# bigai-nlco/VideoTGB

Measured on AMD Instinct MI355X. Metric: clips/sec end-to-end VideoQA (96->8 frames), higher is better.
Workload: dtype bf16; 1 GPU; InstructBLIP-Vicuna-7B + TGB, T=96->8 of 32 frames, 224x224, greedy 16 new tokens (BASELINE.json configs[2]); inputs=resident in HBM when the timed region starts, global_batch=124, parallelism=clip-parallel x1 (no data-path collective), streams=1, weights=seeded N(0,0.02) random init

## Files before the change

include/vtgb.h:

```cpp
#ifndef VTGB_H
#define VTGB_H

#include <stddef.h>
#include <stdint.h>

#ifdef __cplusplus
extern "C" {
#endif

typedef struct ihipStream_t* vtgb_stream_t;

#define VTGB_VERSION 601

#define VTGB_OK 0
#define VTGB_EINVAL (-1)
#define VTGB_EWORKSPACE (-2)
#define VTGB_EHIP (-3)
#define VTGB_EUNSUPPORTED (-4)

#define VTGB_F32 0
#define VTGB_BF16 1
#define VTGB_BF16X3 2
#define VTGB_F16C8 3

// ... 360 lines not shown
    int32_t n_images, H, W;
    int32_t variant;
    int32_t out_kind;
    const void* x;
    const void* weights;
    const float* bias;
    const int32_t* scale;
    const void* resid;
    void* out;
    float* moments;
    void* workspace;
    size_t workspace_bytes;
} vtgb_raft_layer1_h8_args;
size_t vtgb_raft_layer1_h8_workspace_bytes(const vtgb_raft_layer1_h8_args* a);
int vtgb_raft_layer1_h8(const vtgb_raft_layer1_h8_args* a, vtgb_stream_t stream);

typedef struct {
    int32_t dtype, n_pairs, H8, W8, dim;
    int32_t pairs_per_clip, frames_per_clip, first_off, second_off, n_images;
    float scale;
    const float* fmap;
    void* levels[4];
    void* workspace;
    size_t workspace_bytes;
} vtgb_raft_corr_args;
size_t vtgb_raft_corr_workspace_bytes(const vtgb_raft_corr_args* a);
int vtgb_raft_corr(const vtgb_raft_corr_args* a, vtgb_stream_t stream);

#define VTGB_RAFT_ENC_NW 40
typedef struct {
// ... 295 lines not shown
```

videotgb_amd/_lib.py:

```python
from __future__ import annotations

import ctypes as C
import os

import torch

HERE = os.path.dirname(os.path.abspath(__file__))
LIB_PATH = os.environ.get("VTGB_LIB") or os.path.join(HERE, "libvtgb.so")

F32, BF16 = 0, 1
BF16X3 = 2
F16C8 = 3
MAP_A, MAP_B = 0, 1
POOL_MEAN, POOL_CONCAT = 0, 1
TGB_MODE = {"text": 0, "vision": 0, "fusion": 1, "multi_modal": 2}
EPI_STORE, EPI_GELU, EPI_RESID_F32, EPI_STORE_F32 = 0, 1, 2, 3
VIT_NW_GLOBAL, VIT_NW_LAYER = 6, 18
QF_NW_GLOBAL, QF_NW_LAYER = 4, 32
TGB_NW_GLOBAL, TGB_NW_LAYER = 17, 26

EXPORTS = [
    "vtgb_version", "vtgb_last_error", "vtgb_pack_bf16", "vtgb_span_select", "vtgb_span_to_frames",
    "vtgb_gather_frames", "vtgb_vit_patch_kpad", "vtgb_vit_workspace_bytes", "vtgb_vit_forward",
    "vtgb_qformer_workspace_bytes", "vtgb_qformer_forward", "vtgb_pool_project_workspace_bytes",
# ... 7 lines not shown
    "vtgb_gemm_skinny_workspace_bytes", "vtgb_gemm_skinny", "vtgb_pack_skinny_weight_bytes", "vtgb_pack_skinny_weight",
    "vtgb_pack_skinny_weight_fp8_bytes", "vtgb_pack_skinny_weight_fp8", "vtgb_gemm_skinny_fp8", "vtgb_gemm_skinny_bias",
    "vtgb_raft_update_workspace_bytes", "vtgb_raft_update", "vtgb_raft_encoder_workspace_bytes", "vtgb_raft_encoder",
    "vtgb_raft_corr_workspace_bytes", "vtgb_raft_corr", "vtgb_preprocess_frames", "vtgb_concat_text_io", "vtgb_shifted_ce_forward", "vtgb_shifted_ce_backward",
    "vtgb_comm_unique_id", "vtgb_comm_init", "vtgb_comm_destroy", "vtgb_allreduce_f32",
    "vtgb_attn_train_forward", "vtgb_attn_train_backward",
    "vtgb_gemm_train", "vtgb_gemm_train_workspace_bytes", "vtgb_col_sum_parts", "vtgb_col_sum_f32", "vtgb_layernorm_train_partials", "vtgb_layernorm_train_forward", "vtgb_layernorm_train_backward",
    "vtgb_gelu_forward", "vtgb_gelu_backward",
    "vtgb_pair_pack", "vtgb_pair_conv", "vtgb_pair_conv_ex", "vtgb_attention_tiled",
    "vtgb_llm_decode_attention_split_workspace_bytes", "vtgb_llm_decode_attention_split",
    "vtgb_llm_decode_attention_split_fp8", "vtgb_llm_rope_cache_fp8", "vtgb_llm_rope_cache_prefill_fp8",
    "vtgb_raft_lookup_convc1", "vtgb_raft_gru_half", "vtgb_llm_lora", "vtgb_conv_launch", "vtgb_attention_cached",
    "vtgb_llm_decode_attention_beam", "vtgb_llm_beam_candidates", "vtgb_llm_attention_rows_beam", "vtgb_llm_decode_attention_beam_fp8",
    "vtgb_pack_skinny_weight_mxfp4_bytes", "vtgb_pack_skinny_weight_mxfp4", "vtgb_gemm_skinny_mxfp4",
    "vtgb_raft_stem_workspace_bytes", "vtgb_raft_stem", "vtgb_llm_lora_parts", "vtgb_llm_pick_greedy", "vtgb_llm_beam_candidates_eos",
    "vtgb_raft_layer1_h8_workspace_bytes", "vtgb_raft_layer1_h8",
]
COMM_ID_BYTES = 128

i32, i64, f32, vp, sz = C.c_int32, C.c_int64, C.c_float, C.c_void_p, C.c_size_t


class AttnTrainArgs(C.Structure):
    _fields_ = [("batch", i32), ("heads", i32), ("head_dim", i32), ("s_q", i32), ("s_kv", i32), ("q", vp), ("k", vp), ("v", vp),
                ("q_tok", i64), ("kv_tok", i64), ("q_batch", i64), ("kv_batch", i64), ("key_mask", vp), ("drop", vp), ("scale", f32),
                ("out", vp), ("o_tok", i64), ("o_batch", i64), ("lse", vp), ("dout", vp), ("dq", vp), ("dk", vp), ("dv", vp), ("delta", vp)]


class GemmTrainArgs(C.Structure):
    _fields_ = [("compute", i32), ("M", i32), ("N", i32), ("K", i32), ("a", vp), ("lda", i64), ("a_dtype", i32), ("a_kmajor", i32),
                ("b", vp), ("ldb", i64), ("b_dtype", i32), ("b_kmajor", i32), ("bias", vp), ("out", vp), ("ldo", i64), ("workspace", vp), ("workspace_bytes", sz)]
# ... 103 lines not shown
class ConvLaunchArgs(C.Structure):
    _fields_ = [("dtype", i32), ("out_kind", i32), ("site", i32), ("n_images", i32), ("H", i32), ("W", i32), ("KH", i32), ("KW", i32), ("stride", i32),
                ("Hi", i32), ("Wi", i32), ("C1", i32), ("C2", i32), ("N", i32), ("act", i32), ("post_relu", i32), ("out_scale", f32), ("a", vp), ("a2", vp),
                ("weights", vp), ("bias", vp), ("out", vp), ("ld_out", i64), ("moments", vp), ("stats_part", vp), ("stats_part_floats", i64), ("resid", vp),
                ("ld_resid", i64), ("tail_w", vp), ("tail_out", vp)]


class RaftStemArgs(C.Structure):
    _fields_ = [("n_images", i32), ("H", i32), ("W", i32), ("variant", i32), ("out_kind", i32), ("images", vp), ("weights", vp), ("bias", vp), ("out", vp),
                ("moments", vp), ("workspace", vp), ("workspace_bytes", sz)]


class RaftLayer1H8Args(C.Structure):
    _fields_ = [("n_images", i32), ("H", i32), ("W", i32), ("variant", i32), ("out_kind", i32), ("x", vp), ("weights", vp), ("bias", vp), ("scale", vp),
                ("resid", vp), ("out", vp), ("moments", vp), ("workspace", vp), ("workspace_bytes", sz)]


class RaftCorrArgs(C.Structure):
    _fields_ = [("dtype", i32), ("n_pairs", i32), ("H8", i32), ("W8", i32), ("dim", i32), ("pairs_per_clip", i32), ("frames_per_clip", i32),
                ("first_off", i32), ("second_off", i32), ("n_images", i32), ("scale", f32), ("fmap", vp), ("levels", vp * 4),
                ("workspace", vp), ("workspace_bytes", sz)]


class RaftEncoderArgs(C.Structure):
    _fields_ = [("dtype", i32), ("n_images", i32), ("H", i32), ("W", i32), ("norm", i32), ("images", vp), ("weights", C.POINTER(vp)), ("out", vp),
                ("workspace", vp), ("workspace_bytes", sz)]


class GemmSkinnyArgs(C.Structure):
    _fields_ = [("M", i32), ("N", i32), ("K", i32), ("n_splits", i32), ("x", vp), ("ldx", i64), ("w", vp), ("ldw", i64), ("out", vp), ("ldo", i64),
# ... 122 lines not shown
    L.vtgb_pair_conv_ex.restype = C.c_int
    L.vtgb_raft_lookup_convc1.argtypes = [C.POINTER(RaftLookupConvc1Args), vp]
    L.vtgb_raft_lookup_convc1.restype = C.c_int
    L.vtgb_raft_gru_half.argtypes = [C.POINTER(RaftGruHalfArgs), vp]
    L.vtgb_raft_gru_half.restype = C.c_int
    L.vtgb_conv_launch.argtypes = [C.POINTER(ConvLaunchArgs), vp]
    L.vtgb_conv_launch.restype = C.c_int
    L.vtgb_raft_stem.argtypes = [C.POINTER(RaftStemArgs), vp]
    L.vtgb_raft_stem.restype = C.c_int
    L.vtgb_raft_stem_workspace_bytes.argtypes = [C.POINTER(RaftStemArgs)]
    L.vtgb_raft_stem_workspace_bytes.restype = sz
    L.vtgb_raft_layer1_h8.argtypes = [C.POINTER(RaftLayer1H8Args), vp]
    L.vtgb_raft_layer1_h8.restype = C.c_int
    L.vtgb_raft_layer1_h8_workspace_bytes.argtypes = [C.POINTER(RaftLayer1H8Args)]
    L.vtgb_raft_layer1_h8_workspace_bytes.restype = sz
    L.vtgb_raft_update.argtypes = [C.POINTER(RaftUpdateArgs), vp]
    L.vtgb_raft_update.restype = C.c_int
    L.vtgb_raft_update_workspace_bytes.argtypes = [C.POINTER(RaftUpdateArgs)]
    L.vtgb_raft_update_workspace_bytes.restype = sz
    L.vtgb_raft_encoder.argtypes = [C.POINTER(RaftEncoderArgs), vp]
    L.vtgb_raft_encoder.restype = C.c_int
    L.vtgb_raft_encoder_workspace_bytes.argtypes = [C.POINTER(RaftEncoderArgs)]
    L.vtgb_raft_encoder_workspace_bytes.restype = sz
    L.vtgb_raft_corr.argtypes = [C.POINTER(RaftCorrArgs), vp]
    L.vtgb_raft_corr.restype = C.c_int
    L.vtgb_raft_corr_workspace_bytes.argtypes = [C.POINTER(RaftCorrArgs)]
    L.vtgb_raft_corr_workspace_bytes.restype = sz
    L.vtgb_llm_rmsnorm.argtypes = [C.c_int, vp, vp, vp, vp, i64, i32, f32, vp]
    L.vtgb_llm_rope_cache.argtypes = [C.c_int, vp, vp, vp, vp, vp, vp, vp, i32, i32, i32, i32, i32, vp]
    L.vtgb_llm_rope_cache_prefill.argtypes = [C.c_int, vp, vp, vp, vp, vp, i32, i32, i32, i32, i32, i32, vp]
# ... 123 lines not shown
```

videotgb_amd/csrc/common.h:

```cpp
#pragma once
#include <hip/hip_runtime.h>
#include <stdint.h>
#include <stdio.h>

#include "vtgb.h"

typedef __bf16 bf16_t;
typedef __attribute__((ext_vector_type(8))) __bf16 bf16x8;
typedef __attribute__((ext_vector_type(4))) __bf16 bf16x4;
typedef __attribute__((ext_vector_type(4))) float f32x4;

#if defined(__HIPCC__)
__device__ __forceinline__ float bf16_round(float v) {
    unsigned u = __float_as_uint(v);
    if ((u & 0x7F800000u) != 0x7F800000u) u += 0x7FFFu + ((u >> 16) & 1u);
    return __uint_as_float(u & 0xFFFF0000u);
}
#endif

void vtgb_set_error(const char* fmt, ...);

#define VTGB_REQUIRE(cond, code, ...)  \
    do {                               \
        if (!(cond)) {                 \
// ... 146 lines not shown
bool stem7x7_supported(int H, int W);
int launch_stem7x7(const float* img, const void* w, const float* bias, float* out_f32, float* stats, float* stats_part, void* out_bf16, int n_img, int H, int W,
                   int relu, hipStream_t s);
int launch_stem7x7_x3(const float* img, const void* w, const float* bias, float* out_f32, float* stats, float* stats_part, void* out_pair, int h8, int n_img, int H,
                      int W, hipStream_t s);
size_t conv64_stats_part_floats(int n_img);
int launch_stats_finish_tiles(const float* part, float* stats, int n_img, int HW, int N, int64_t M, hipStream_t s);
int launch_stats_finish_parts(const float* part, float* stats, int n_img, int parts, int C, hipStream_t s);
int cu_count();

bool conv3x3_c64_supported(int H, int W);
int launch_conv3x3_c64(const void* in, const void* w, const float* bias, float* out_f32, float* stats, float* stats_part, void* out_bf16, const void* resid,
                       int n_img, int H, int W, int relu, int post_relu, hipStream_t s);
bool layer1_h8_supported(int H, int W);
int launch_layer1_h8(const void* in, const void* w, const float* bias, const int* scale, float* out_f32, void* out_pair, const void* resid, int out_bf16, int n_img, int H,
                     int W, hipStream_t s);

struct LnDesc {
    int dtype, M, D;
    float eps;
    const float* x;
    int64_t ldx;
    RowMap x_map;
    const float* gamma;
    const float* beta;
    float* out_f32;
    void* out_act;
    int64_t ldo;
    RowMap o_map;
};
int launch_layernorm(const LnDesc& d, hipStream_t s);
// ... 27 lines not shown
```

videotgb_amd/csrc/conv64.hip:

```cpp
#include <type_traits>
#include <utility>
#include "common.h"
#include "pair_h8.h"

namespace {

constexpr int C64_R = 8, C64_RS = 128;
constexpr int C64_ROW_BYTES = C64_RS * 128;
constexpr int C64_LDS = C64_R * C64_ROW_BYTES + 8 * 32 * 2 * 4 + 64 * 4;
typedef __attribute__((address_space(3))) void* c64_lptr_t;

struct Conv64Params {
    const bf16_t* in;
    const bf16_t* w;
    const float* bias;
    float* out_f32;
    float* stats;
    float* stats_part;
    bf16_t* out_bf16;
    const bf16_t* resid;
    int n_img, H, W, relu, post_relu;
    int parts, rows_per_part;
};

// ... 414 lines not shown
typedef _Float16 l1_f16x8 __attribute__((ext_vector_type(8)));

template <class F, int... G>
__device__ __forceinline__ void l1_static_for(std::integer_sequence<int, G...>, F&& f) { (f(std::integral_constant<int, G>{}), ...); }

struct Layer1H8Params {
    const char* in;
    const char* w;
    const float* bias;
    const int* scale;
    float* out_f32;
    char* out_pair;
    const char* resid;
    int n_img, H, W, out_bf16;
    int parts, rows_per_part, row_bytes;
};

template <int MODE, int OBF>
__global__ __launch_bounds__(512) void layer1_h8_kernel(const Layer1H8Params p) {
#if defined(__HIP_DEVICE_COMPILE__)
    extern __shared__ __attribute__((aligned(16))) char ring[];
    const int tid = threadIdx.x, lane = tid & 63, fr = lane & 15, fg = lane >> 4;
    const int wave = __builtin_amdgcn_readfirstlane(tid >> 6);
    const int wn = wave & 3, wm = wave >> 2;
    const int H = p.H, W = p.W, row_bytes = p.row_bytes;
    const int sc_w = *p.scale;

    l1_i32x4 wh[9][2];
    l1_i32x8 wc[9];
    {
        const char* const wrow = p.w + (wn * 16 + fr) * 2304 + fg * 16;
#pragma unroll
        for (int t = 0; t < 9; t++) {
            wh[t][0] = *reinterpret_cast<const l1_i32x4*>(wrow + t * 128);
            wh[t][1] = *reinterpret_cast<const l1_i32x4*>(wrow + t * 128 + 64);
            wc[t].lo = *reinterpret_cast<const l1_i32x4*>(wrow + (9 + t) * 128);
            wc[t].hi = *reinterpret_cast<const l1_i32x4*>(wrow + (9 + t) * 128 + 64);
        }
    }
    float* const bias_s = reinterpret_cast<float*>(ring + (L1_R - 1) * row_bytes + L1_READ_SPAN);
    if (tid < 64) bias_s[tid] = p.bias[tid];
    __syncthreads();

    constexpr unsigned OOB = 0x80000000u;
    const int n_pieces = row_bytes >> 10;
    const int dma_x = wave * 4 + (lane >> 4) - 1;
    const unsigned dma_off0 = (unsigned)(dma_x * 256 + (((lane & 15) ^ ((dma_x + 1) & 15)) << 4));
    unsigned x_off[3];
#pragma unroll
    for (int kx = 0; kx < 3; kx++) {
        const int slot = wm * 64 + fr + kx;
        x_off[kx] = (unsigned)(slot * 256 + ((fg ^ (slot & 15)) << 4));
    }
    const int nj = W - wm * 64 >= 64 ? 4 : W - wm * 64 <= 0 ? 0 : (W - wm * 64 + 15) >> 4;
    typedef __attribute__((__vector_size__(4 * sizeof(unsigned)))) unsigned u32x4_t;
    typedef __attribute__((__vector_size__(2 * sizeof(unsigned)))) unsigned u32x2_t;
    constexpr int OPX = 256;
// ... 7 lines not shown
        if (y0 >= H) continue;
        const int y1 = y0 + p.rows_per_part < H ? y0 + p.rows_per_part : H;
        const int64_t ioff = (int64_t)img * H * W * 256;
        const auto rsrc = __builtin_amdgcn_make_buffer_rsrc(const_cast<char*>(p.in + ioff), 0, H * W * 256, 0x00020000);
        const auto orsrc = __builtin_amdgcn_make_buffer_rsrc(MODE == 0 ? (void*)(reinterpret_cast<char*>(p.out_f32) + ioff) : (void*)(p.out_pair + ioff), 0, H * W * OPX, 0x00020000);
        const auto rrsrc = __builtin_amdgcn_make_buffer_rsrc(const_cast<char*>((MODE == 2 ? p.resid : p.in) + ioff), 0, H * W * 256, 0x00020000);
#define L1_ISSUE(yy)                                                                                                          \
        {                                                                                                                      \
            const int so_ = ((yy) >= 0 && (yy) < H) ? (yy) * W * 256 : 0x7FFFFF00;        \
            char* const dst_ = ring + ((yy) & (L1_R - 1)) * row_bytes + wave * 1024;                                           \
            _Pragma("unroll") for (int q = 0; q < 4; q++)                                                                      \
                if (q * 8 + wave < n_pieces)                                                                                   \
                    __builtin_amdgcn_raw_ptr_buffer_load_lds(rsrc, (c64_lptr_t)(dst_ + q * 8192), 16,                          \
                                                             (dma_x + q * 32 >= 0 && dma_x + q * 32 < W) ? dma_off0 + q * 8192u : OOB, so_, 0, 0); \
        }
        __builtin_amdgcn_s_waitcnt(0x0F70);
        __builtin_amdgcn_s_barrier();
        L1_ISSUE(y0 - 1)
        L1_ISSUE(y0)
        L1_ISSUE(y0 + 1)
        auto step = [&](auto nj_c, const int y) {
            constexpr int NJ = decltype(nj_c)::value;
            constexpr int NST = (MODE == 0 ? 1 : 2) * NJ;
            if (y == y0) __builtin_amdgcn_s_waitcnt(0x0F70);
            else __builtin_amdgcn_s_waitcnt(0x0F70 | NST);
            __builtin_amdgcn_s_barrier();
            u32x2_t rh[NJ], rl[NJ];
            if constexpr (MODE == 2) {
#pragma unroll
                for (int jj = 0; jj < NJ; jj++) {
                    const unsigned off = px0 + jj * 16 < W ? o_off0 + (unsigned)(jj * 16 * OPX + y * W * 256) : OOB;
                    rh[jj] = __builtin_bit_cast(u32x2_t, __builtin_amdgcn_raw_buffer_load_b64(rrsrc, off, 0, 0));
                    rl[jj] = __builtin_bit_cast(u32x2_t, __builtin_amdgcn_raw_buffer_load_b64(rrsrc, off != OOB ? off + 128u : OOB, 0, 0));
                }
            }
            L1_ISSUE(y + 2)
            f32x4 acc[NJ];
#pragma unroll
            for (int jj = 0; jj < NJ; jj++) acc[jj] = *reinterpret_cast<const f32x4*>(bias_s + wn * 16 + fg * 4);
            l1_i32x4 xg[3][NJ];
// ... 48 lines not shown
                        hu = __builtin_bit_cast(u32x2_t, hi); lu = __builtin_bit_cast(u32x2_t, lo);
                    } else {
                        h8_split4(v, hu, lu);
                    }
                    __builtin_amdgcn_raw_buffer_store_b64(hu, orsrc, off, 0, 0);
                    __builtin_amdgcn_raw_buffer_store_b64(lu, orsrc, ok ? off + 128u : OOB, 0, 0);
                }
            }
        };
        if (nj == 3) {
            for (int y = y0; y < y1; y++) step(std::integral_constant<int, 3>{}, y);
        } else {
            for (int y = y0; y < y1; y++) step(std::integral_constant<int, 4>{}, y);
        }
#undef L1_ISSUE
    }
#endif
}

}

bool conv3x3_c64_supported(int H, int W) { return W >= 16 && W <= C64_RS - 2 && H >= 1; }

size_t conv64_stats_part_floats(int n_img) { return ((size_t)n_img + 4 * (size_t)cu_count()) * 2 * 64 * 2; }

int launch_conv3x3_c64(const void* in, const void* w, const float* bias, float* out_f32, float* stats, float* stats_part, void* out_bf16, const void* resid,
                       int n_img, int H, int W, int relu, int post_relu, hipStream_t s) {
    VTGB_REQUIRE(conv3x3_c64_supported(H, W), VTGB_EUNSUPPORTED, "conv3x3_c64: W=%d outside [16, %d]", W, C64_RS - 2);
    VTGB_REQUIRE((int64_t)H * W * 128 < 0x7FFFFF00ll, VTGB_EUNSUPPORTED, "conv3x3_c64: image too large");
    Conv64Params p;
// ... 67 lines not shown
}

int launch_stem7x7(const float* img, const void* w, const float* bias, float* out_f32, float* stats, float* stats_part, void* out_bf16, int n_img, int H, int W,
                   int relu, hipStream_t s) {
    return stem7x7_launch(false, img, w, bias, out_f32, stats, stats_part, out_bf16, 0, n_img, H, W, relu, s);
}
int launch_stem7x7_x3(const float* img, const void* w, const float* bias, float* out_f32, float* stats, float* stats_part, void* out_pair, int h8, int n_img, int H,
                      int W, hipStream_t s) {
    VTGB_REQUIRE((out_f32 != nullptr) != (out_pair != nullptr), VTGB_EINVAL, "stem7x7 x3: exactly one of the fp32 rows and the pair rows");
    return stem7x7_launch(true, img, w, bias, out_f32, stats, stats_part, out_pair, h8, n_img, H, W, out_pair ? 1 : 0, s);
}

bool layer1_h8_supported(int H, int W) { return W >= 16 && W <= L1_MAX_W && H >= 4 && (int64_t)H * W * 256 < 0x7FFFFF00ll; }

int launch_layer1_h8(const void* in, const void* w, const float* bias, const int* scale, float* out_f32, void* out_pair, const void* resid, int out_bf16, int n_img, int H,
                     int W, hipStream_t s) {
    VTGB_REQUIRE(n_img > 0 && layer1_h8_supported(H, W), VTGB_EUNSUPPORTED, "layer1_h8: %d images of %d x %d outside 16 <= W <= %d, H >= 4", n_img, H, W, L1_MAX_W);
    VTGB_REQUIRE(in && w && bias && scale && ((out_f32 != nullptr) != (out_pair != nullptr)) && (!resid || out_pair) && (!out_bf16 || resid), VTGB_EINVAL,
                 "layer1_h8: operands, the scale byte and exactly one of the fp32 rows and the pair rows (resid belongs to pair rows, bf16 pairs to the residual tail)");
    Layer1H8Params p;
    p.in = (const char*)in; p.w = (const char*)w; p.bias = bias; p.scale = scale; p.out_f32 = out_f32; p.out_pair = (char*)out_pair; p.resid = (const char*)resid;
    p.n_img = n_img; p.H = H; p.W = W; p.out_bf16 = out_bf16;
    p.row_bytes = ((W + 2 + 3) / 4) * 1024;
    int parts = 1;
    while ((int64_t)n_img * parts < 4 * cu_count() && H / (parts * 2) >= 7) parts *= 2;
    p.rows_per_part = (H + parts - 1) / parts;
    p.parts = (H + p.rows_per_part - 1) / p.rows_per_part;
    const int64_t units = (int64_t)n_img * p.parts;
    const int grid = units < cu_count() ? (int)units : cu_count();
    const int lds = (L1_R - 1) * p.row_bytes + L1_READ_SPAN + 256;
    constexpr int lds_max = (L1_R - 1) * ((L1_MAX_W + 2 + 3) / 4) * 1024 + L1_READ_SPAN + 256;
    const double flops = 2.0 * n_img * H * W * 64.0 * 576.0;
    ProfScope prof(VTGB_PROF_CONV, flops, s, 2.0 * flops);
    static DeviceOnce a0, a1, a2, a3;
    if (out_f32) {
        VTGB_FUNC_LDS_ONCE(a0, (layer1_h8_kernel<0, 0>), lds_max);
        hipLaunchKernelGGL((layer1_h8_kernel<0, 0>), dim3(grid), dim3(512), lds, s, p);
    } else if (!resid) {
        VTGB_FUNC_LDS_ONCE(a1, (layer1_h8_kernel<1, 0>), lds_max);
        hipLaunchKernelGGL((layer1_h8_kernel<1, 0>), dim3(grid), dim3(512), lds, s, p);
    } else if (!out_bf16) {
        VTGB_FUNC_LDS_ONCE(a2, (layer1_h8_kernel<2, 0>), lds_max);
        hipLaunchKernelGGL((layer1_h8_kernel<2, 0>), dim3(grid), dim3(512), lds, s, p);
    } else {
        VTGB_FUNC_LDS_ONCE(a3, (layer1_h8_kernel<2, 1>), lds_max);
        hipLaunchKernelGGL((layer1_h8_kernel<2, 1>), dim3(grid), dim3(512), lds, s, p);
    }
    VTGB_HIP(hipGetLastError());
    return VTGB_OK;
}
// ... 1 lines not shown
```

videotgb_amd/csrc/raft_enc.hip:

```cpp
#include <math.h>
#include <string.h>

#include "common.h"
#include "conv_descs.h"

template <typename T>
__global__ __launch_bounds__(256) void raft_stem_pack_kernel(const float* __restrict__ img, T* __restrict__ out, T* __restrict__ pad_page,
                                                             int64_t n_px, int H, int W) {
    constexpr bool PAIR = sizeof(T) == 2;
    constexpr int CP = PAIR ? 128 : 64;
    const int64_t i = (int64_t)blockIdx.x * blockDim.x + threadIdx.x;
    if (i < 64) pad_page[i] = (T)0.f;
    if (i >= n_px * 4) return;
    const int64_t px_i = i >> 2;
    const int dX = (int)(i & 3), W2 = W >> 1, H2 = H >> 1;
    const int X = (int)(px_i % W2), Y = (int)((px_i / W2) % H2);
    const int64_t n = px_i / ((int64_t)W2 * H2);
    T v[12], l[12];
#pragma unroll
    for (int py = 0; py < 2; py++)
#pragma unroll
        for (int pxx = 0; pxx < 2; pxx++) {
            const int col = 2 * (X + dX - 2) + pxx, row = 2 * Y + py;
            const bool ok = (unsigned)col < (unsigned)W;
// ... 223 lines not shown
    d.algo_flops = 2.0 * (double)M2 * 64 * 147;
    VTGB_TRY(launch_conv_gemm(d, s));
    if (t.pair) return launch_x3_pair_pass(t.cf, 64, nullptr, HW, nullptr, 128, 64, t.pair, 128, 64, 64, 64, 1, 0, M2, s, t.h8);
    if (sf) return launch_stats_finish_tiles(sf, t.stats, t.n, HW, 64, M2, s);
    const int splits = HW >= 4096 ? 16 : HW >= 1024 ? 4 : 1;
    hipLaunchKernelGGL(inorm_stats_kernel, dim3(t.n, splits), dim3(256), 0, s, t.cf, t.spart, HW, 64, 64);
    return launch_stats_finish_parts(t.spart, t.stats, t.n, splits, 64, s);
}

struct EncH8 {
    const void* A; const void* W; const float* bias; const int* scale;
    int n, H, Wd, C, Cpad;
    float* cf; float* spart; float* stats;
    void* pair; const void* resid; int out_bf16;
    void* zero;
};
static int g_l1_h8 = 3;
extern "C" void vtgb_debug_set_l1_h8(int mask) { g_l1_h8 = mask & 3; }
static int enc_conv_h8(const EncH8& t, int variant, hipStream_t s) {
    const int HW = t.H * t.Wd, C2 = 2 * t.Cpad;
    const int64_t Mo = (int64_t)t.n * HW;
    if (variant != 0) {
        VTGB_REQUIRE(t.C == 64 && t.Cpad == 64 && layer1_h8_supported(t.H, t.Wd), VTGB_EUNSUPPORTED, "enc_conv_h8: the row-resident kernel takes 64 -> 64 channels, 16 <= W <= 112, H >= 4");
        VTGB_REQUIRE(variant == 1 || (!t.pair && t.spart && HW >= 256), VTGB_EINVAL, "enc_conv_h8: tile-order moments belong to fp32 rows of images of >= 256 pixels");
        VTGB_TRY(launch_layer1_h8(t.A, t.W, t.bias, t.scale, t.pair ? nullptr : t.cf, t.pair, t.resid, t.out_bf16, t.n, t.H, t.Wd, s));
        if (variant == 1) return VTGB_OK;
        hipLaunchKernelGGL(stats_tiles_c64_kernel, dim3((unsigned)((Mo + 255) / 256)), dim3(512), 0, s, t.cf, t.spart, (int)Mo, HW);
        return launch_stats_finish_tiles(t.spart, t.stats, t.n, HW, 64, Mo, s);
    }
    GemmDesc d;
    memset(&d, 0, sizeof(d));
    d.dtype = VTGB_BF16; d.M = (int)Mo; d.K = 9 * C2;
    d.A = t.A; d.lda = C2; d.W = t.W; d.ldw = d.K; d.bias = t.bias;
    d.conv_H = t.H; d.conv_W = t.Wd; d.conv_KH = 3; d.conv_KW = 3; d.conv_Cin = C2; d.conv_split = C2; d.zero_page = t.zero;
    d.h8_run = 9 * (t.Cpad / 64); d.h8_scale = t.scale;
    d.algo_flops = 2.0 * Mo * (double)t.C * (9 * t.C);
    if (!t.pair) {
        d.N = t.C; d.epi = VTGB_EPI_STORE_F32; d.out = t.cf; d.ldo = t.Cpad;
        d.col_stats = t.spart; d.stats_rows = HW;
        VTGB_TRY(launch_conv_h8(d, s));
        if (t.spart) VTGB_TRY(launch_stats_finish_tiles(t.spart, t.stats, t.n, HW, t.C, Mo, s));
        return VTGB_OK;
    }
    d.N = t.Cpad; d.epi = VTGB_EPI_SPLIT; d.act = 1; d.out = t.pair; d.ldo = C2; d.split_lo = t.Cpad;
// ... 138 lines not shown
        } else if (!inorm && !x3) {
            VTGB_TRY(conv_bn(Mo, g, 3, Cin_pad, g.stride, Hi, Wi, x, bw[0], F(bw[1]), 1, nullptr, 0, t1));
            const void* res = x;
            outb = t2;
            if (g.stride != 1) {
                VTGB_TRY(conv_bn(Mo, g, 1, Cin_pad, g.stride, Hi, Wi, x, bw[4], F(bw[5]), 0, nullptr, 0, t2));
                res = t2;
                outb = x;
            }
            VTGB_TRY(conv_bn(Mo, g, 3, g.Cpad, 1, g.Ho, g.Wo, t1, bw[2], F(bw[3]), 1, res, 1, outb));
        } else if (h8l1) {
            VTGB_REQUIRE(w[40], VTGB_EINVAL, "raft_encoder: weights[40] (the f16c8 convolutions' scale bytes) is NULL at VTGB_F16C8");
            const int C2 = 2 * g.Cpad;
            const bool s2 = g.stride != 1;
            const bool l1 = g.C == 64 && g.Cpad == 64 && !s2 && layer1_h8_supported(g.Ho, g.Wo);
            auto conv_h8 = [&](const void* A, const void* Wt, const float* bias, float* col_stats, int si) -> int {
                const EncH8 t{A, Wt, bias, (const int*)w[40] + si, n, g.Ho, g.Wo, g.C, g.Cpad, cf, col_stats, stats, nullptr, nullptr, 0, zero};
                return enc_conv_h8(t, l1 && (g_l1_h8 & 2) ? (col_stats ? 2 : 1) : 0, s);
            };
            auto conv_pair = [&](const void* A, const void* Wt, const float* bias, int si, const void* resid, void* out, int out_bf16) -> int {
                const EncH8 t{A, Wt, bias, (const int*)w[40] + si, n, g.Ho, g.Wo, g.C, g.Cpad, nullptr, nullptr, nullptr, out, resid, out_bf16, zero};
                return enc_conv_h8(t, l1 && (g_l1_h8 & 1) && (resid || !out_bf16) ? 1 : 0, s);
            };
            const int out_h8 = (b & 1) == 0;
            if (!inorm) {
                auto split_conv = [&](int K, const void* Wt, const float* bias, int relu, void* out) -> int {
                    GemmDesc d = enc_conv(dt, (int)Mo, g.Cpad, g.Ho, g.Wo, K, Cin_pad, g.stride, Hi, Wi, x, Wt, bias, nullptr, C2, zero, nullptr);
                    d.epi = VTGB_EPI_SPLIT; d.act = relu; d.out = out; d.split_lo = g.Cpad; d.split_f16c8 = 1;
                    d.algo_flops = 2.0 * Mo * (double)g.C * (K * K * Cin_pad);
                    return launch_conv_gemm(d, s);
                };
                if (s2) VTGB_TRY(split_conv(3, bw[0], F(bw[1]), 1, t1));
                else VTGB_TRY(conv_pair(x, bw[0], F(bw[1]), 2 * b, nullptr, t1, 0));
                const void* res = x;
                outb = t2;
                if (s2) {
                    VTGB_TRY(split_conv(1, bw[4], F(bw[5]), 0, t2));
                    res = t2;
                    outb = x;
                }
                VTGB_TRY(conv_pair(t1, bw[2], F(bw[3]), 2 * b + 1, res, outb, !out_h8));
            } else {
                float* sf = stats_for(stats, HWo, g.C);
                if (s2) VTGB_TRY(conv_stats(enc_conv(dt, (int)Mo, g.C, g.Ho, g.Wo, 3, Cin_pad, g.stride, Hi, Wi, x, bw[0], F(bw[1]), cf, g.Cpad, zero, sf), stats));
                else VTGB_TRY(conv_h8(x, bw[0], F(bw[1]), sf, 2 * b));
                VTGB_TRY(norm(cf, Mo, HWo, g.C, g.Cpad, g.Cpad, nullptr, t1, 1, 0, stats, sf != nullptr, 1));
                sf = stats_for(stats, HWo, g.C);
                VTGB_TRY(conv_h8(t1, bw[2], F(bw[3]), sf, 2 * b + 1));
                const void* res = x;
                if (s2) {
                    float* sf2 = stats_for(stats2, HWo, g.C);
                    VTGB_TRY(conv_stats(enc_conv(dt, (int)Mo, g.C, g.Ho, g.Wo, 1, Cin_pad, g.stride, Hi, Wi, x, bw[4], F(bw[5]), cf2, g.Cpad, zero, sf2), stats2));
                    VTGB_TRY(norm(cf2, Mo, HWo, g.C, g.Cpad, g.Cpad, nullptr, t2, 0, 0, stats2, sf2 != nullptr));
                    res = t2;
                }
                outb = t1;
                VTGB_TRY(norm(cf, Mo, HWo, g.C, g.Cpad, g.Cpad, res, outb, 1, 1, stats, sf != nullptr, out_h8, !s2));
            }
        } else if (x3 && !inorm && g.Cpad == 128) {
            auto split_conv = [&](int K, int Cin, int stride, int Hi_, int Wi_, const void* A, const void* Wt, const float* bias, int relu, void* out) -> int {
                GemmDesc d = enc_conv(dt, (int)Mo, g.Cpad, g.Ho, g.Wo, K, Cin, stride, Hi_, Wi_, A, Wt, bias, nullptr, 2 * g.Cpad, zero, nullptr);
                d.epi = VTGB_EPI_SPLIT; d.act = relu; d.out = out; d.split_lo = g.Cpad;
                d.algo_flops = 2.0 * Mo * (double)g.C * (K * K * Cin);
                return launch_conv_gemm(d, s);
            };
            VTGB_TRY(split_conv(3, Cin_pad, g.stride, Hi, Wi, x, bw[0], F(bw[1]), 1, t1));
            VTGB_TRY(launch_conv_gemm(enc_conv(dt, (int)Mo, g.C, g.Ho, g.Wo, 3, g.Cpad, 1, g.Ho, g.Wo, t1, bw[2], F(bw[3]), cf, g.Cpad, zero, nullptr), s));
            const void* res = x;
            outb = t1;
            if (g.stride != 1) {
                VTGB_TRY(split_conv(1, Cin_pad, g.stride, Hi, Wi, x, bw[4], F(bw[5]), 0, t2));
                res = t2;
// ... 112 lines not shown
}
extern "C" size_t vtgb_raft_layer1_h8_workspace_bytes(const vtgb_raft_layer1_h8_args* a) {
    Workspace ws(nullptr, 0);
    if (layer1_unit_impl(a, ws, nullptr) != VTGB_OK) return 0;
    return align_up(ws.used, 256);
}
extern "C" int vtgb_raft_layer1_h8(const vtgb_raft_layer1_h8_args* a, vtgb_stream_t stream) {
    VTGB_REQUIRE(a, VTGB_EINVAL, "raft_layer1_h8: NULL args");
    Workspace probe(nullptr, 0);
    VTGB_TRY(layer1_unit_impl(a, probe, nullptr));
    VTGB_REQUIRE(a->workspace, VTGB_EWORKSPACE, "raft_layer1_h8: workspace is NULL (%zu bytes needed)", align_up(probe.used, 256));
    Workspace ws(a->workspace, a->workspace_bytes);
    return layer1_unit_impl(a, ws, (hipStream_t)stream);
}

extern "C" size_t vtgb_raft_encoder_workspace_bytes(const vtgb_raft_encoder_args* a) {
    Workspace ws(nullptr, 0);
    if (enc_impl(a, ws, nullptr) != VTGB_OK) return 0;
    return align_up(ws.used, 256);
}
extern "C" int vtgb_raft_encoder(const vtgb_raft_encoder_args* a, vtgb_stream_t stream) {
    VTGB_REQUIRE(a && a->workspace, VTGB_EWORKSPACE, "raft_encoder: workspace is NULL");
    Workspace ws(a->workspace, a->workspace_bytes);
    return enc_impl(a, ws, stream);
}
```

videotgb_amd/ops.py:

```python
from __future__ import annotations

import ctypes as C
import logging
import math
from typing import Dict, List, Optional, Sequence, Tuple

import torch

from . import _lib as L
from ._lib import BF16, BF16X3, F16C8, F32

_log = logging.getLogger("videotgb_amd")
_ws_logged = set()


def _log_workspace(what: str, need: int, detail: str) -> None:
    key = (what, need >> 30)
    if key in _ws_logged:
        return
    _ws_logged.add(key)
    _log.log(logging.WARNING if need > (64 << 30) else logging.INFO, "%s: %.2f GB of workspace (%s)", what, need / 2 ** 30, detail)

Tensor = torch.Tensor

# ... 1427 lines not shown
    assert out.is_contiguous() and out.numel() >= M * (128 if pair else 64) and out.dtype == (torch.int16 if pair else torch.float32)
    mom = torch.empty(n, 64, 2, dtype=torch.float32, device=dev) if moments else None
    a = L.RaftLayer1H8Args(n, H, W, variant, out_kind, x.data_ptr(), packed.data_ptr(), bias_t.data_ptr(), scale.data_ptr(), _ptr(resid), out.data_ptr(), _ptr(mom),
                           None, 0)
    need = L.lib().vtgb_raft_layer1_h8_workspace_bytes(C.byref(a))
    if need == 0:
        L.check(L.lib().vtgb_raft_layer1_h8(C.byref(a), _stream()))
    ws = workspace if workspace is not None else _ws.get(need, dev)
    assert ws.numel() >= need
    a.workspace, a.workspace_bytes = ws.data_ptr(), ws.numel()
    L.check(L.lib().vtgb_raft_layer1_h8(C.byref(a), _stream()))
    torch.cuda.current_stream().synchronize()
    return (out, mom) if moments else out


class RaftEncoderWeights(_WeightTable):

    def __init__(self, sd: Dict[str, Tensor], prefix: str, batch_norm: bool, code: int = BF16):
        super().__init__(code)
        self.batch_norm = batch_norm
        p = prefix

        def folded(conv, bn):
            w, b = sd[p + conv + ".weight"].float(), sd[p + conv + ".bias"].float()
            if batch_norm:
                g = sd[p + bn + ".weight"].float() / torch.sqrt(sd[p + bn + ".running_var"].float() + 1e-5)
                w = w * g.view(-1, 1, 1, 1)
                b = (b - sd[p + bn + ".running_mean"].float()) * g + sd[p + bn + ".bias"].float()
            return w, b

# ... 72 lines not shown
```

Before: 38.50 clips/s.

## Fuse instance-norm+ReLU of layer1 input into row-resident h8 conv kernel

Adds an FIN variant of the layer1 h8 conv kernel that reads fp32 input rows and applies instance-norm and ReLU in LDS from per-image moments, then splits into h8 pairs before the MMA. In the RAFT encoder's layer1 residual blocks, this replaces the separate norm pass and its bf16-pair intermediate write between the two 3x3 convs. It also adds a standalone h8n entry point and a debug toggle. The cost is extra LDS conversion work and barriers inside the conv loop, plus reading fp32 rows, which are twice as large, through DMA.

```diff
diff --git a/include/vtgb.h b/include/vtgb.h
--- a/include/vtgb.h
+++ b/include/vtgb.h
@@ -398,6 +398,28 @@
 } vtgb_raft_layer1_h8_args;
 size_t vtgb_raft_layer1_h8_workspace_bytes(const vtgb_raft_layer1_h8_args* a);
 int vtgb_raft_layer1_h8(const vtgb_raft_layer1_h8_args* a, vtgb_stream_t stream);
+
+#define VTGB_L1_IN_PAIR 0
+#define VTGB_L1_IN_F32 1
+typedef struct {
+    int32_t n_images, H, W;
+    int32_t variant;
+    int32_t in_kind;
+    int32_t fuse;
+    int32_t out_kind;
+    const void* x;
+    const float* x_moments;
+    const void* weights;
+    const float* bias;
+    const int32_t* scale;
+    const void* resid;
+    void* out;
+    float* moments;
+    void* workspace;
+    size_t workspace_bytes;
+} vtgb_raft_layer1_h8n_args;
+size_t vtgb_raft_layer1_h8n_workspace_bytes(const vtgb_raft_layer1_h8n_args* a);
+int vtgb_raft_layer1_h8n(const vtgb_raft_layer1_h8n_args* a, vtgb_stream_t stream);
 
 typedef struct {
     int32_t dtype, n_pairs, H8, W8, dim;
diff --git a/videotgb_amd/_lib.py b/videotgb_amd/_lib.py
--- a/videotgb_amd/_lib.py
+++ b/videotgb_amd/_lib.py
@@ -45,7 +45,7 @@
     "vtgb_llm_decode_attention_beam", "vtgb_llm_beam_candidates", "vtgb_llm_attention_rows_beam", "vtgb_llm_decode_attention_beam_fp8",
     "vtgb_pack_skinny_weight_mxfp4_bytes", "vtgb_pack_skinny_weight_mxfp4", "vtgb_gemm_skinny_mxfp4",
     "vtgb_raft_stem_workspace_bytes", "vtgb_raft_stem", "vtgb_llm_lora_parts", "vtgb_llm_pick_greedy", "vtgb_llm_beam_candidates_eos",
-    "vtgb_raft_layer1_h8_workspace_bytes", "vtgb_raft_layer1_h8",
+    "vtgb_raft_layer1_h8_workspace_bytes", "vtgb_raft_layer1_h8", "vtgb_raft_layer1_h8n_workspace_bytes", "vtgb_raft_layer1_h8n",
 ]
 COMM_ID_BYTES = 128
 
@@ -179,6 +179,14 @@
 class RaftLayer1H8Args(C.Structure):
     _fields_ = [("n_images", i32), ("H", i32), ("W", i32), ("variant", i32), ("out_kind", i32), ("x", vp), ("weights", vp), ("bias", vp), ("scale", vp),
                 ("resid", vp), ("out", vp), ("moments", vp), ("workspace", vp), ("workspace_bytes", sz)]
+
+
+L1_IN_PAIR, L1_IN_F32 = 0, 1
+
+
+class RaftLayer1H8NArgs(C.Structure):
+    _fields_ = [("n_images", i32), ("H", i32), ("W", i32), ("variant", i32), ("in_kind", i32), ("fuse", i32), ("out_kind", i32), ("x", vp), ("x_moments", vp),
+                ("weights", vp), ("bias", vp), ("scale", vp), ("resid", vp), ("out", vp), ("moments", vp), ("workspace", vp), ("workspace_bytes", sz)]
 
 
 class RaftCorrArgs(C.Structure):
@@ -331,6 +339,12 @@
     L.vtgb_raft_layer1_h8.restype = C.c_int
     L.vtgb_raft_layer1_h8_workspace_bytes.argtypes = [C.POINTER(RaftLayer1H8Args)]
     L.vtgb_raft_layer1_h8_workspace_bytes.restype = sz
+    L.vtgb_raft_layer1_h8n.argtypes = [C.POINTER(RaftLayer1H8NArgs), vp]
+    L.vtgb_raft_layer1_h8n.restype = C.c_int
+    L.vtgb_raft_layer1_h8n_workspace_bytes.argtypes = [C.POINTER(RaftLayer1H8NArgs)]
+    L.vtgb_raft_layer1_h8n_workspace_bytes.restype = sz
+    L.vtgb_debug_set_l1_norm.argtypes = [C.c_int]
+    L.vtgb_debug_set_l1_norm.restype = None
     L.vtgb_raft_update.argtypes = [C.POINTER(RaftUpdateArgs), vp]
     L.vtgb_raft_update.restype = C.c_int
     L.vtgb_raft_update_workspace_bytes.argtypes = [C.POINTER(RaftUpdateArgs)]
diff --git a/videotgb_amd/csrc/common.h b/videotgb_amd/csrc/common.h
--- a/videotgb_amd/csrc/common.h
+++ b/videotgb_amd/csrc/common.h
@@ -184,7 +184,7 @@
                        int n_img, int H, int W, int relu, int post_relu, hipStream_t s);
 bool layer1_h8_supported(int H, int W);
 int launch_layer1_h8(const void* in, const void* w, const float* bias, const int* scale, float* out_f32, void* out_pair, const void* resid, int out_bf16, int n_img, int H,
-                     int W, hipStream_t s);
+                     int W, hipStream_t s, const float* in_stats = nullptr);
 
 struct LnDesc {
     int dtype, M, D;
diff --git a/videotgb_amd/csrc/conv64.hip b/videotgb_amd/csrc/conv64.hip
--- a/videotgb_amd/csrc/conv64.hip
+++ b/videotgb_amd/csrc/conv64.hip
@@ -452,9 +452,27 @@
     const char* resid;
     int n_img, H, W, out_bf16;
     int parts, rows_per_part, row_bytes;
+    const float* in_stats;
 };
 
-template <int MODE, int OBF>
+__device__ __forceinline__ void l1_norm_entry(const float sum, const float sumsq, const float inv, const bool upper, float& a, float& rstd) {
+#pragma clang fp contract(off)
+    const float mean = inv * sum, q = inv * sumsq;
+    const float var = upper ? __builtin_fmaf(-mean, mean, q) : q - mean * mean;
+    a = upper ? mean : sum;
+    rstd = rsqrtf(fmaxf(var, 0.f) + 1e-5f);
+}
+__device__ __forceinline__ f32x4 l1_norm4(const f32x4 x, const f32x4 n01, const f32x4 n23, const float inv) {
+#pragma clang fp contract(off)
+    f32x4 y;
+    y[0] = fmaxf(__builtin_fmaf(-inv, n01[0], x[0]) * n01[1], 0.f);
+    y[1] = fmaxf(__builtin_fmaf(-inv, n01[2], x[1]) * n01[3], 0.f);
+    y[2] = fmaxf((x[2] - n23[0]) * n23[1], 0.f);
+    y[3] = fmaxf((x[3] - n23[2]) * n23[3], 0.f);
+    return y;
+}
+
+template <int MODE, int OBF, int FIN = 0>
 __global__ __launch_bounds__(512) void layer1_h8_kernel(const Layer1H8Params p) {
 #if defined(__HIP_DEVICE_COMPILE__)
     extern __shared__ __attribute__((aligned(16))) char ring[];
@@ -479,6 +497,9 @@
     float* const bias_s = reinterpret_cast<float*>(ring + (L1_R - 1) * row_bytes + L1_READ_SPAN);
     if (tid < 64) bias_s[tid] = p.bias[tid];
     __syncthreads();
+    float* const nrm_s = bias_s + 64;
+    float inv_hw = 0.f;
+    if constexpr (FIN) inv_hw = __builtin_bit_cast(float, __builtin_amdgcn_readfirstlane(__builtin_bit_cast(int, 1.0f / (float)(H * W))));
 
     constexpr unsigned OOB = 0x80000000u;
     const int n_pieces = row_bytes >> 10;
@@ -516,16 +537,52 @@
                     __builtin_amdgcn_raw_ptr_buffer_load_lds(rsrc, (c64_lptr_t)(dst_ + q * 8192), 16,                          \
                                                              (dma_x + q * 32 >= 0 && dma_x + q * 32 < W) ? dma_off0 + q * 8192u : OOB, so_, 0, 0); \
         }
-        __builtin_amdgcn_s_waitcnt(0x0F70);
+        if constexpr (FIN) {
+            if (tid < 64) {
+                float a_, rstd_;
+                l1_norm_entry(p.in_stats[((int64_t)img * 64 + tid) * 2], p.in_stats[((int64_t)img * 64 + tid) * 2 + 1], inv_hw, (tid & 2) != 0, a_, rstd_);
+                nrm_s[tid * 2] = a_;
+                nrm_s[tid * 2 + 1] = rstd_;
+            }
+            __builtin_amdgcn_s_waitcnt(0x0070);
+        } else {
+            __builtin_amdgcn_s_waitcnt(0x0F70);
+        }
         __builtin_amdgcn_s_barrier();
         L1_ISSUE(y0 - 1)
         L1_ISSUE(y0)
         L1_ISSUE(y0 + 1)
+#define L1_CONVERT(yy)                                                                                                        \
+        if ((yy) >= 0 && (yy) < H) {                                                                                           \
+                                                        \
+            const int sw_ = (dma_x + 1) & 15, j_ = (lane & 15) ^ sw_;           \
+            char* const slot_ = ring + ((yy) & (L1_R - 1)) * row_bytes + wave * 1024 + (lane >> 4) * 256;                      \
+            f32x4 cv_[4];                                                                                                      \
+            _Pragma("unroll") for (int q = 0; q < 4; q++)                                                                      \
+                if (q * 8 + wave < n_pieces) cv_[q] = *reinterpret_cast<const f32x4*>(slot_ + q * 8192 + (lane & 15) * 16);    \
+            const f32x4 n01 = *reinterpret_cast<const f32x4*>(nrm_s + j_ * 8), n23 = *reinterpret_cast<const f32x4*>(nrm_s + j_ * 8 + 4); \
+            _Pragma("unroll") for (int q = 0; q < 4; q++)                                                                      \
+                if (q * 8 + wave < n_pieces && dma_x + q * 32 >= 0 && dma_x + q * 32 < W) {                                    \
+                    const f32x4 v = l1_norm4(cv_[q], n01, n23, inv_hw);                                                        \
+                    u32x2_t hu, lu;                                                                                            \
+                    h8_split4(v, hu, lu);                                                                                      \
+                    *reinterpret_cast<u32x2_t*>(slot_ + q * 8192 + (((j_ >> 1) ^ sw_) << 4) + (j_ & 1) * 8) = hu;              \
+                    *reinterpret_cast<u32x2_t*>(slot_ + q * 8192 + (((8 + (j_ >> 1)) ^ sw_) << 4) + (j_ & 1) * 8) = lu;        \
+                }                                                                                                              \
+        }
         auto step = [&](auto nj_c, const int y) {
             constexpr int NJ = decltype(nj_c)::value;
             constexpr int NST = (MODE == 0 ? 1 : 2) * NJ;
             if (y == y0) __builtin_amdgcn_s_waitcnt(0x0F70);
             else __builtin_amdgcn_s_waitcnt(0x0F70 | NST);
+            if constexpr (FIN) {
+                if (y == y0) {
+                    L1_CONVERT(y - 1)
+                    L1_CONVERT(y)
+                }
+                L1_CONVERT(y + 1)
+                __builtin_amdgcn_s_waitcnt(0xC07F);
+            }
             __builtin_amdgcn_s_barrier();
             u32x2_t rh[NJ], rl[NJ];
             if constexpr (MODE == 2) {
@@ -604,6 +661,7 @@
             for (int y = y0; y < y1; y++) step(std::integral_constant<int, 4>{}, y);
         }
 #undef L1_ISSUE
+#undef L1_CONVERT
     }
 #endif
 }
@@ -701,13 +759,15 @@
 bool layer1_h8_supported(int H, int W) { return W >= 16 && W <= L1_MAX_W && H >= 4 && (int64_t)H * W * 256 < 0x7FFFFF00ll; }
 
 int launch_layer1_h8(const void* in, const void* w, const float* bias, const int* scale, float* out_f32, void* out_pair, const void* resid, int out_bf16, int n_img, int H,
-                     int W, hipStream_t s) {
+                     int W, hipStream_t s, const float* in_stats) {
     VTGB_REQUIRE(n_img > 0 && layer1_h8_supported(H, W), VTGB_EUNSUPPORTED, "layer1_h8: %d images of %d x %d outside 16 <= W <= %d, H >= 4", n_img, H, W, L1_MAX_W);
     VTGB_REQUIRE(in && w && bias && scale && ((out_f32 != nullptr) != (out_pair != nullptr)) && (!resid || out_pair) && (!out_bf16 || resid), VTGB_EINVAL,
                  "layer1_h8: operands, the scale byte and exactly one of the fp32 rows and the pair rows (resid belongs to pair rows, bf16 pairs to the residual tail)");
+    VTGB_REQUIRE(!in_stats || out_f32, VTGB_EUNSUPPORTED, "layer1_h8: fp32 input rows (normalised in the kernel) are built for fp32 output rows only");
+    VTGB_REQUIRE(!in_stats || (const void*)out_f32 != in, VTGB_EINVAL, "layer1_h8: the fp32 output rows cannot be the fp32 input rows");
     Layer1H8Params p;
     p.in = (const char*)in; p.w = (const char*)w; p.bias = bias; p.scale = scale; p.out_f32 = out_f32; p.out_pair = (char*)out_pair; p.resid = (const char*)resid;
-    p.n_img = n_img; p.H = H; p.W = W; p.out_bf16 = out_bf16;
+    p.n_img = n_img; p.H = H; p.W = W; p.out_bf16 = out_bf16; p.in_stats = in_stats;
     p.row_bytes = ((W + 2 + 3) / 4) * 1024;
     int parts = 1;
     while ((int64_t)n_img * parts < 4 * cu_count() && H / (parts * 2) >= 7) parts *= 2;
@@ -715,12 +775,15 @@
     p.parts = (H + p.rows_per_part - 1) / p.rows_per_part;
     const int64_t units = (int64_t)n_img * p.parts;
     const int grid = units < cu_count() ? (int)units : cu_count();
-    const int lds = (L1_R - 1) * p.row_bytes + L1_READ_SPAN + 256;
-    constexpr int lds_max = (L1_R - 1) * ((L1_MAX_W + 2 + 3) / 4) * 1024 + L1_READ_SPAN + 256;
+    const int lds = (L1_R - 1) * p.row_bytes + L1_READ_SPAN + 256 + (in_stats ? 512 : 0);
+    constexpr int lds_max = (L1_R - 1) * ((L1_MAX_W + 2 + 3) / 4) * 1024 + L1_READ_SPAN + 256 + 512;
     const double flops = 2.0 * n_img * H * W * 64.0 * 576.0;
     ProfScope prof(VTGB_PROF_CONV, flops, s, 2.0 * flops);
-    static DeviceOnce a0, a1, a2, a3;
-    if (out_f32) {
+    static DeviceOnce a0, a1, a2, a3, a4;
+    if (in_stats) {
+        VTGB_FUNC_LDS_ONCE(a4, (layer1_h8_kernel<0, 0, 1>), lds_max);
+        hipLaunchKernelGGL((layer1_h8_kernel<0, 0, 1>), dim3(grid), dim3(512), lds, s, p);
+    } else if (out_f32) {
         VTGB_FUNC_LDS_ONCE(a0, (layer1_h8_kernel<0, 0>), lds_max);
         hipLaunchKernelGGL((layer1_h8_kernel<0, 0>), dim3(grid), dim3(512), lds, s, p);
     } else if (!resid) {
diff --git a/videotgb_amd/csrc/raft_enc.hip b/videotgb_amd/csrc/raft_enc.hip
--- a/videotgb_amd/csrc/raft_enc.hip
+++ b/videotgb_amd/csrc/raft_enc.hip
@@ -261,20 +261,24 @@
     float* cf; float* spart; float* stats;
     void* pair; const void* resid; int out_bf16;
     void* zero;
+    const float* a_stats;
 };
 static int g_l1_h8 = 3;
 extern "C" void vtgb_debug_set_l1_h8(int mask) { g_l1_h8 = mask & 3; }
+static int g_l1_norm = 3;
+extern "C" void vtgb_debug_set_l1_norm(int mask) { g_l1_norm = mask & 3; }
 static int enc_conv_h8(const EncH8& t, int variant, hipStream_t s) {
     const int HW = t.H * t.Wd, C2 = 2 * t.Cpad;
     const int64_t Mo = (int64_t)t.n * HW;
     if (variant != 0) {
         VTGB_REQUIRE(t.C == 64 && t.Cpad == 64 && layer1_h8_supported(t.H, t.Wd), VTGB_EUNSUPPORTED, "enc_conv_h8: the row-resident kernel takes 64 -> 64 channels, 16 <= W <= 112, H >= 4");
         VTGB_REQUIRE(variant == 1 || (!t.pair && t.spart && HW >= 256), VTGB_EINVAL, "enc_conv_h8: tile-order moments belong to fp32 rows of images of >= 256 pixels");
-        VTGB_TRY(launch_layer1_h8(t.A, t.W, t.bias, t.scale, t.pair ? nullptr : t.cf, t.pair, t.resid, t.out_bf16, t.n, t.H, t.Wd, s));
+        VTGB_TRY(launch_layer1_h8(t.A, t.W, t.bias, t.scale, t.pair ? nullptr : t.cf, t.pair, t.resid, t.out_bf16, t.n, t.H, t.Wd, s, t.a_stats));
         if (variant == 1) return VTGB_OK;
         hipLaunchKernelGGL(stats_tiles_c64_kernel, dim3((unsigned)((Mo + 255) / 256)), dim3(512), 0, s, t.cf, t.spart, (int)Mo, HW);
         return launch_stats_finish_tiles(t.spart, t.stats, t.n, HW, 64, Mo, s);
     }
+    VTGB_REQUIRE(!t.a_stats, VTGB_EUNSUPPORTED, "enc_conv_h8: the implicit GEMM stages through DMA and cannot normalise fp32 input rows");
     GemmDesc d;
     memset(&d, 0, sizeof(d));
     d.dtype = VTGB_BF16; d.M = (int)Mo; d.K = 9 * C2;
@@ -443,8 +447,8 @@
             const int C2 = 2 * g.Cpad;
             const bool s2 = g.stride != 1;
             const bool l1 = g.C == 64 && g.Cpad == 64 && !s2 && layer1_h8_supported(g.Ho, g.Wo);
-            auto conv_h8 = [&](const void* A, const void* Wt, const float* bias, float* col_stats, int si) -> int {
-                const EncH8 t{A, Wt, bias, (const int*)w[40] + si, n, g.Ho, g.Wo, g.C, g.Cpad, cf, col_stats, stats, nullptr, nullptr, 0, zero};
+            auto conv_h8 = [&](const void* A, const void* Wt, const float* bias, float* col_stats, int si, const float* a_stats = nullptr, float* out = nullptr) -> int {
+                const EncH8 t{A, Wt, bias, (const int*)w[40] + si, n, g.Ho, g.Wo, g.C, g.Cpad, out ? out : cf, col_stats, stats, nullptr, nullptr, 0, zero, a_stats};
                 return enc_conv_h8(t, l1 && (g_l1_h8 & 2) ? (col_stats ? 2 : 1) : 0, s);
             };
             auto conv_pair = [&](const void* A, const void* Wt, const float* bias, int si, const void* resid, void* out, int out_bf16) -> int {
@@ -473,9 +477,16 @@
                 float* sf = stats_for(stats, HWo, g.C);
                 if (s2) VTGB_TRY(conv_stats(enc_conv(dt, (int)Mo, g.C, g.Ho, g.Wo, 3, Cin_pad, g.stride, Hi, Wi, x, bw[0], F(bw[1]), cf, g.Cpad, zero, sf), stats));
                 else VTGB_TRY(conv_h8(x, bw[0], F(bw[1]), sf, 2 * b));
-                VTGB_TRY(norm(cf, Mo, HWo, g.C, g.Cpad, g.Cpad, nullptr, t1, 1, 0, stats, sf != nullptr, 1));
-                sf = stats_for(stats, HWo, g.C);
-                VTGB_TRY(conv_h8(t1, bw[2], F(bw[3]), sf, 2 * b + 1));
+                const bool fin = l1 && (g_l1_h8 & 2) && (g_l1_norm & 2) && sf != nullptr;
+                float* c2 = cf;
+                if (fin) {
+                    c2 = (float*)t1;
+                    VTGB_TRY(conv_h8(cf, bw[2], F(bw[3]), sf, 2 * b + 1, stats, c2));
+                } else {
+                    VTGB_TRY(norm(cf, Mo, HWo, g.C, g.Cpad, g.Cpad, nullptr, t1, 1, 0, stats, sf != nullptr, 1));
+                    sf = stats_for(stats, HWo, g.C);
+                    VTGB_TRY(conv_h8(t1, bw[2], F(bw[3]), sf, 2 * b + 1));
+                }
                 const void* res = x;
                 if (s2) {
                     float* sf2 = stats_for(stats2, HWo, g.C);
@@ -483,8 +494,8 @@
                     VTGB_TRY(norm(cf2, Mo, HWo, g.C, g.Cpad, g.Cpad, nullptr, t2, 0, 0, stats2, sf2 != nullptr));
                     res = t2;
                 }
-                outb = t1;
-                VTGB_TRY(norm(cf, Mo, HWo, g.C, g.Cpad, g.Cpad, res, outb, 1, 1, stats, sf != nullptr, out_h8, !s2));
+                outb = fin ? t2 : t1;
+                VTGB_TRY(norm(c2, Mo, HWo, g.C, g.Cpad, g.Cpad, res, outb, 1, 1, stats, sf != nullptr, out_h8, !s2));
             }
         } else if (x3 && !inorm && g.Cpad == 128) {
             auto split_conv = [&](int K, int Cin, int stride, int Hi_, int Wi_, const void* A, const void* Wt, const float* bias, int relu, void* out) -> int {
@@ -627,6 +638,65 @@
     return layer1_unit_impl(a, ws, (hipStream_t)stream);
 }
 
+static int layer1n_unit_impl(const vtgb_raft_layer1_h8n_args* a, Workspace& ws, hipStream_t s) {
+    VTGB_REQUIRE(a, VTGB_EINVAL, "raft_layer1_h8n: NULL args");
+    VTGB_REQUIRE(a->n_images > 0 && a->H >= 1 && a->W >= 1 && a->variant >= 0 && a->variant <= 2 && (a->fuse == 0 || a->fuse == 1), VTGB_EINVAL,
+                 "raft_layer1_h8n: bad dims n=%d H=%d W=%d variant=%d fuse=%d", a->n_images, a->H, a->W, a->variant, a->fuse);
+    const int ok = a->out_kind;
+    VTGB_REQUIRE(ok == VTGB_CONV_OUT_F32 || ok == VTGB_CONV_OUT_PAIR_BF16 || ok == VTGB_CONV_OUT_PAIR_F16C8, VTGB_EINVAL,
+                 "raft_layer1_h8n: bad out_kind %d (VTGB_CONV_OUT_F32, _PAIR_BF16 or _PAIR_F16C8)", ok);
+    VTGB_REQUIRE(a->in_kind == VTGB_L1_IN_PAIR || a->in_kind == VTGB_L1_IN_F32, VTGB_EINVAL, "raft_layer1_h8n: bad in_kind %d (VTGB_L1_IN_PAIR or VTGB_L1_IN_F32)", a->in_kind);
+    const bool pair = ok != VTGB_CONV_OUT_F32, fin = a->in_kind == VTGB_L1_IN_F32;
+    const int HW = a->H * a->W;
+    const int64_t M = (int64_t)a->n_images * HW;
+    VTGB_REQUIRE(M < (1ll << 31) / 64, VTGB_EUNSUPPORTED, "raft_layer1_h8n: too many pixels per call (chunk the images)");
+    VTGB_REQUIRE(fin == (a->x_moments != nullptr), VTGB_EINVAL, "raft_layer1_h8n: x_moments belong to fp32 input rows, and fp32 input rows need them");
+    VTGB_REQUIRE(fin || a->fuse == 0, VTGB_EINVAL, "raft_layer1_h8n: fuse belongs to fp32 input rows");
+    VTGB_REQUIRE(pair || !a->resid, VTGB_EINVAL, "raft_layer1_h8n: resid belongs to pair rows");
+    VTGB_REQUIRE(ok != VTGB_CONV_OUT_PAIR_BF16 || a->resid, VTGB_EINVAL, "raft_layer1_h8n: bf16 pairs are the output of the residual tail (resid is NULL)");
+    VTGB_REQUIRE(a->variant != 2 || (!pair && HW >= 256 && a->moments), VTGB_EINVAL,
+                 "raft_layer1_h8n: variant 2 (tile-order moments) belongs to fp32 rows of images of >= 256 pixels, with moments");
+    VTGB_REQUIRE(a->variant != 1 || !a->moments, VTGB_EINVAL, "raft_layer1_h8n: variant 1 writes no moments (moments must be NULL)");
+    VTGB_REQUIRE(!a->moments || (!pair && HW >= 256), VTGB_EINVAL, "raft_layer1_h8n: moments belong to fp32 rows of images of >= 256 pixels");
+    VTGB_REQUIRE(a->variant == 0 || layer1_h8_supported(a->H, a->W), VTGB_EUNSUPPORTED,
+                 "raft_layer1_h8n: the row-resident kernel does not take %d x %d images (16 <= W <= 112, H >= 4; variant 0 does)", a->H, a->W);
+    VTGB_REQUIRE(!a->fuse || (a->variant != 0 && !pair), VTGB_EUNSUPPORTED,
+                 "raft_layer1_h8n: fp32 input rows are normalised in the row-resident kernel (variants 1, 2) for fp32 output rows only (fuse 0 takes the rest)");
+    float* spart = a->moments ? (float*)ws.take((size_t)(M / 256 + 2) * 128 * 4 * 4) : nullptr;
+    void* zero = ws.take(256);
+    void* y = fin && !a->fuse ? ws.take((size_t)M * 256) : nullptr;
+    if (ws.dry) return VTGB_OK;
+    VTGB_REQUIRE(ws.ok(), VTGB_EWORKSPACE, "raft_layer1_h8n: workspace %zu < %zu bytes", ws.size, ws.used);
+    VTGB_REQUIRE(a->x && a->weights && a->bias && a->scale && a->out, VTGB_EINVAL, "raft_layer1_h8n: NULL operand");
+    VTGB_REQUIRE(a->out != a->x, VTGB_EINVAL, "raft_layer1_h8n: out must not be x");
+    auto al16 = [](const void* p) { return ((uintptr_t)p & 15) == 0; };
+    VTGB_REQUIRE(al16(a->x) && al16(a->x_moments) && al16(a->weights) && al16(a->bias) && al16(a->out) && al16(a->resid) && al16(a->moments) && al16(a->workspace) &&
+                     ((uintptr_t)a->scale & 3) == 0,
+                 VTGB_EINVAL, "raft_layer1_h8n: misaligned operand (16 bytes; the scale: 4)");
+    VTGB_HIP(hipMemsetAsync(zero, 0, 256, s));
+    const void* A = a->x;
+    if (y) {
+        VTGB_TRY(launch_x3_pair_pass((const float*)a->x, 64, a->x_moments, HW, nullptr, 128, 64, y, 128, 64, 64, 64, 1, 0, M, s, 1, 0));
+        A = y;
+    }
+    const EncH8 t{A, a->weights, a->bias, (const int*)a->scale, a->n_images, a->H, a->W, 64, 64, pair ? nullptr : (float*)a->out, spart, a->moments,
+                  pair ? a->out : nullptr, a->resid, ok == VTGB_CONV_OUT_PAIR_BF16, zero, a->fuse ? a->x_moments : nullptr};
+    return enc_conv_h8(t, a->variant, s);
+}
+extern "C" size_t vtgb_raft_layer1_h8n_workspace_bytes(const vtgb_raft_layer1_h8n_args* a) {
+    Workspace ws(nullptr, 0);
+    if (layer1n_unit_impl(a, ws, nullptr) != VTGB_OK) return 0;
+    return align_up(ws.used, 256);
+}
+extern "C" int vtgb_raft_layer1_h8n(const vtgb_raft_layer1_h8n_args* a, vtgb_stream_t stream) {
+    VTGB_REQUIRE(a, VTGB_EINVAL, "raft_layer1_h8n: NULL args");
+    Workspace probe(nullptr, 0);
+    VTGB_TRY(layer1n_unit_impl(a, probe, nullptr));
+    VTGB_REQUIRE(a->workspace, VTGB_EWORKSPACE, "raft_layer1_h8n: workspace is NULL (%zu bytes needed)", align_up(probe.used, 256));
+    Workspace ws(a->workspace, a->workspace_bytes);
+    return layer1n_unit_impl(a, ws, (hipStream_t)stream);
+}
+
 extern "C" size_t vtgb_raft_encoder_workspace_bytes(const vtgb_raft_encoder_args* a) {
     Workspace ws(nullptr, 0);
     if (enc_impl(a, ws, nullptr) != VTGB_OK) return 0;
diff --git a/videotgb_amd/ops.py b/videotgb_amd/ops.py
--- a/videotgb_amd/ops.py
+++ b/videotgb_amd/ops.py
@@ -1465,6 +1465,33 @@
     return (out, mom) if moments else out
 
 
+def raft_layer1_h8n(x: Tensor, x_moments: Tensor, w: Tensor, bias: Tensor, n: int, H: int, W: int, fuse: int = 1, variant: int = 1, moments: bool = False,
+                    out: Optional[Tensor] = None):
+    _need_cuda(x, w)
+    dev = x.device
+    M = n * H * W
+    assert x.is_contiguous() and x.dtype == torch.float32 and tuple(x.shape) == (M, 64) and tuple(w.shape) == (64, 3, 3, 64)
+    assert x_moments.is_contiguous() and x_moments.dtype == torch.float32 and tuple(x_moments.shape) == (n, 64, 2)
+    sw, byte = h8_weight_scale(w)
+    packed = h8_conv_pack(w.to(dev), sw)
+    scale = torch.tensor([byte], dtype=torch.int32, device=dev)
+    bias_t = bias.to(dev).contiguous().float()
+    if out is None:
+        out = torch.empty(M, 64, dtype=torch.float32, device=dev)
+    assert out.is_contiguous() and out.numel() >= M * 64 and out.dtype == torch.float32
+    mom = torch.empty(n, 64, 2, dtype=torch.float32, device=dev) if moments else None
+    a = L.RaftLayer1H8NArgs(n, H, W, variant, L.L1_IN_F32, fuse, L.CONV_OUT_F32, x.data_ptr(), x_moments.data_ptr(), packed.data_ptr(), bias_t.data_ptr(),
+                            scale.data_ptr(), None, out.data_ptr(), _ptr(mom), None, 0)
+    need = L.lib().vtgb_raft_layer1_h8n_workspace_bytes(C.byref(a))
+    if need == 0:
+        L.check(L.lib().vtgb_raft_layer1_h8n(C.byref(a), _stream()))
+    ws = _ws.get(need, dev)
+    a.workspace, a.workspace_bytes = ws.data_ptr(), ws.numel()
+    L.check(L.lib().vtgb_raft_layer1_h8n(C.byref(a), _stream()))
+    torch.cuda.current_stream().synchronize()
+    return (out, mom) if moments else out
+
+
 class RaftEncoderWeights(_WeightTable):
 
     def __init__(self, sd: Dict[str, Tensor], prefix: str, batch_norm: bool, code: int = BF16):
```

After: 38.75 clips/s (median of 6 runs). No clear change (+0.7%).
